# XinMing0411/AC-VAE

Hardware: AMD Instinct MI355X
Metric: train-step captions/s (and audio-sec/s) at B=32, 1/2/4/8 MI355X (higher is better)
Workload: dtype f32

## Files before the change

### acvae_amd/_lib.py

```python
import ctypes
import os
import re
import threading

import numpy as np
import torch

_HERE = os.path.dirname(os.path.abspath(__file__))
HEADER = os.path.join(os.path.dirname(_HERE), "include", "acvae_hip.h")
LIB_PATH = os.path.join(_HERE, "libacvae_hip.so")

_CT = {"int": ctypes.c_int, "int64_t": ctypes.c_int64, "float": ctypes.c_float, "double": ctypes.c_double,
       "uint64_t": ctypes.c_uint64}
ERRORS = {-1: "ACVAE_EINVAL (bad dims / null pointer)", -2: "ACVAE_EALIGN (alignment)",
          -3: "ACVAE_EUNSUPPORTED", -4: "ACVAE_EWORKSPACE (workspace too small)"}


def parse_header(path=HEADER):
    src = open(path).read()
    src = re.sub(r"/\*.*?\*/", "", src, flags=re.S)
    protos = {}
    for m in re.finditer(r"\b(int|int64_t)\s+(acvae_\w+)\s*\(([^)]*)\)\s*;", src):
        ret, name, args = m.group(1), m.group(2), m.group(3).strip()
        alist = []
# ... 3 lines not shown
                if "*" in a:
                    alist.append((a.split("*")[-1].strip(), ctypes.c_void_p))
                else:
                    toks = a.replace("const ", "").split()
                    alist.append((toks[-1], _CT[toks[0]]))
        protos[name] = (_CT[ret], alist)
    enums = {}
    for m in re.finditer(r"enum\s+\w*\s*\{([^}]*)\}", src):
        val = -1
        for item in m.group(1).split(","):
            item = item.strip()
            if not item:
                continue
            if "=" in item:
                k, v = item.split("=")
                val = int(v.strip(), 0)
                enums[k.strip()] = val
            else:
                val += 1
                enums[item] = val
    return protos, enums


PROTOS, ENUMS = parse_header()
_defs = dict(re.findall(r"#define\s+(ACVAE_\w+)\s+(\d+)", open(HEADER).read()))
ENUMS_TEXT_N = int(_defs["ACVAE_TEXT_NPARAMS"])
ENC_NPARAMS = int(_defs["ACVAE_ENC_NPARAMS"])
ENC_BF16 = int(_defs["ACVAE_ENC_BF16"])
FLAG_NO_PERSIST = int(_defs["ACVAE_FLAG_NO_PERSIST"])
FLAG_DEFER_PARAM_GRADS = int(_defs["ACVAE_FLAG_DEFER_PARAM_GRADS"])
FLAG_NO_ATTN_SPLIT = int(_defs["ACVAE_FLAG_NO_ATTN_SPLIT"])
FLAG_TEST_STALL = int(_defs["ACVAE_FLAG_TEST_STALL"])
FLAG_ROLLOUT_GRAD = int(_defs["ACVAE_FLAG_ROLLOUT_GRAD"])
_lib = None


class options:
    persist = os.environ.get("ACVAE_DECODE_PERSIST", "1") != "0"
    defer = os.environ.get("ACVAE_DECODE_DEFER", "1") != "0"
    attn_split = True
    test_stall = False


class override:
    _lock = threading.Lock()
    _open = []
    _base = None

    def __init__(self, **kw):
        self.kw = kw

    @staticmethod
    def _apply():
        vals = dict(override._base)
        for o in override._open:
            vals.update(o.kw)
        for k, v in vals.items():
            setattr(options, k, v)

    def __enter__(self):
        with override._lock:
            if not override._open:
                override._base = {k: v for k, v in vars(options).items() if not k.startswith("_")}
            override._open.append(self)
            override._apply()
        return self

    def __exit__(self, *exc):
        with override._lock:
            override._open.remove(self)
            override._apply()
        return False

# ... 180 lines not shown
```

### acvae_amd/csrc/decoder.hip

```cpp
#include <cstdlib>
#include <vector>
#include "common.h"
#include "conv.h"
#include "rnn.h"
#include "decode_persist.h"
#include "../../include/acvae_hip.h"

namespace {

struct Bump {
  long off = 0;
  long take(long n) { const long o = off; off = (off + n + 63) & ~63L; return o; }
};

struct Ctx {
  hipStream_t s;
  float* skws;
  operator hipStream_t() const { return s; }
};
inline int gemm(const float* A, long lda, const float* B, long ldb, const float* bias, float* C, long ldc, int M, int N,
                int K, int acc, const Ctx& st) {
  return acvae_gemm_nt_dual(A, lda, B, ldb, K, nullptr, 0, nullptr, 0, 0, bias, C, ldc, M, N, acc, st.s, st.skws);
}
inline int gemm2(const float* A1, long lda1, const float* B1, long ldb1, int K1, const float* A2, long lda2,
                 const float* B2, long ldb2, int K2, const float* bias, float* C, long ldc, int M, int N, int acc,
                 const Ctx& st) {
  if (M <= 64)
    return acvae_gemm_nt_dual(A1, lda1, B1, ldb1, K1, A2, lda2, B2, ldb2, K2, bias, C, ldc, M, N, acc, st.s, st.skws);
  ACVAE_TRY(acvae_gemm_nt_dual(A1, lda1, B1, ldb1, K1, nullptr, 0, nullptr, 0, 0, bias, C, ldc, M, N, acc, st.s, st.skws));
  return acvae_gemm_nt_dual(A2, lda2, B2, ldb2, K2, nullptr, 0, nullptr, 0, 0, nullptr, C, ldc, M, N, 1, st.s, st.skws);
}
struct TnWs { float* p; long bytes; };
inline int gemm_tn(const float* A, long lda, const float* B, long ldb, float* C, long ldc, int M, int N, int K, TnWs ws,
                   hipStream_t st) {
  return acvae_gemm_tn_fused(A, lda, B, ldb, C, ldc, M, N, K, 0, ws.p, ws.bytes, st);
}
inline void zb_skinny(acvae::ZeroBatch& zb, float* skws) { zb.add(skws, acvae_skinny_ticket_words()); }
inline void zb_colsum(acvae::ZeroBatch& zb, double* dpart) { zb.add(dpart, acvae::colsum_ticket_words()); }
inline void zb_tn(acvae::ZeroBatch& zb, TnWs ws) { zb.add(ws.p, TN_TICKETS); }
inline int transp(const float* in, long ld_in, float* out, long ld_out, int rows, int cols, hipStream_t st) {
  return acvae_transpose(in, ld_in, out, ld_out, rows, cols, st);
}
inline int zero(float* p, long n, hipStream_t st) {
  return hipMemsetAsync(p, 0, (size_t)n * sizeof(float), st) == hipSuccess ? ACVAE_OK : (int)hipGetLastError();
}
struct Fork {
  hipStream_t main_s, aux;
  bool on() const { return aux != main_s; }
  static int edge(hipStream_t from, hipStream_t to) {
    constexpr int RING = 64;
    struct Ring { hipEvent_t ev[RING]; int next; int dev; };
    static thread_local Ring ring = {{}, 0, -1};
    int dev = -1;
    if (hipGetDevice(&dev) != hipSuccess) return (int)hipGetLastError();
    if (dev != ring.dev) {
      for (int i = 0; i < RING; ++i) ring.ev[i] = nullptr;
      ring.next = 0; ring.dev = dev;
    }
    hipEvent_t& e = ring.ev[ring.next];
    ring.next = (ring.next + 1) % RING;
    if (!e && hipEventCreateWithFlags(&e, hipEventDisableTiming) != hipSuccess) return (int)hipGetLastError();
    hipError_t r = hipEventRecord(e, from);
    if (r == hipSuccess) r = hipStreamWaitEvent(to, e, 0);
    return r == hipSuccess ? ACVAE_OK : (int)r;
  }
  int begin() const { return on() ? edge(main_s, aux) : ACVAE_OK; }
  int join() const { return on() ? edge(aux, main_s) : ACVAE_OK; }
};
inline long tn_ws_floats(int M, int N, int K) { return acvae_gemm_tn_workspace_bytes(M, N, K) / 4 + 64 + TN_TICKETS; }

enum {
  TP_DEC_EMB, TP_DEC_WIH, TP_DEC_WHH, TP_DEC_BIH, TP_DEC_BHH, TP_DEC_CLS_W, TP_DEC_CLS_B, TP_DEC_ATT_V, TP_DEC_ATT_W,
  TP_DEC_ATT_B, TP_Q_EMB, TP_Q_WIH, TP_Q_WHH, TP_Q_BIH, TP_Q_BHH, TP_Q_WIH_R, TP_Q_WHH_R, TP_Q_BIH_R, TP_Q_BHH_R,
  TP_Q_TML_W, TP_Q_TML_B, TP_P_EMB, TP_P_ATT_V, TP_P_ATT_W, TP_P_ATT_B, TP_P_WIH, TP_P_WHH, TP_P_BIH, TP_P_BHH,
  TP_P_ML_W, TP_P_ML_B, TP_MLO_W, TP_MLO_B, TP_LN_W, TP_LN_B, TP_COUNT
};
static_assert(TP_COUNT == ACVAE_TEXT_NPARAMS, "text parameter table out of sync with the header");

constexpr int POST_MAX_LAYERS = 16;
struct PostLayout {
  long words, x, hidden[POST_MAX_LAYERS], save_f[POST_MAX_LAYERS], save_r[POST_MAX_LAYERS], hprev_f[POST_MAX_LAYERS],
      hprev_r[POST_MAX_LAYERS], argmax, saved_total;
  long gi_f, gi_r, gh, hf, ml, dml, dhid, dgi_f, dgi_r, dgh_f, dgh_r, dh_a, dh_b, dx, wt, wt2, wt_ih0, wt_ih1, wt_ml, pq_hbuf, pq_cnt, tn, dpart, skws,
       dhid2, wtu_hh0, wtu_hh1, wtu_ih0, wtu_ih1, scratch_total;
  long tn_floats, dpart_doubles, pq_cnt_words;
};
int post_layout(int N, int Tc, int E, int Hq, int V, int NL, PostLayout& L) {
  if (N <= 0 || Tc <= 0 || E <= 0 || Hq <= 0 || V <= 0 || NL < 1 || NL > POST_MAX_LAYERS) return ACVAE_EINVAL;
  const long R = (long)N * Tc;
  Bump s;
  L.words = s.take(R * 2);
  L.x = s.take(R * E);
  for (int k = 0; k < NL; ++k) {
    L.hidden[k] = s.take(R * 2 * Hq);
    L.save_f[k] = s.take(R * 4 * Hq); L.save_r[k] = s.take(R * 4 * Hq);
    L.hprev_f[k] = s.take(R * Hq); L.hprev_r[k] = s.take(R * Hq);
  }
  L.argmax = s.take((long)N * 2 * Hq);
  L.saved_total = s.off;
  Bump c;
  L.gi_f = c.take(R * 3 * Hq); L.gi_r = c.take(R * 3 * Hq);
// ... 1234 lines not shown
```

### acvae_amd/csrc/encoder.hip

```cpp
#include <algorithm>
#include "common.h"
#include "conv.h"
#include "resnet.h"
#include "../../include/acvae_hip.h"

namespace {

constexpr int kMaxBlocks = 6;
constexpr int kArchMask = 0xff;
constexpr int kChan[kMaxBlocks + 1] = {1, 64, 128, 256, 512, 1024, 2048};
struct Arch { int blocks; bool pool_last; };
inline bool arch_of(int arch, Arch& a) {
  if (arch & ~(kArchMask | ACVAE_ENC_BF16)) return false;
  if ((arch & kArchMask) == ACVAE_ARCH_CNN10) { a = {4, true}; return true; }
  if ((arch & kArchMask) == ACVAE_ARCH_CNN14_16K) { a = {6, false}; return true; }
  return false;
}
inline bool is_bf16(int arch) { return (arch & ACVAE_ENC_BF16) != 0; }
inline bool wino_on() {
  static const bool on = !getenv("ACVAE_CONV_WINO") || atoi(getenv("ACVAE_CONV_WINO")) != 0;
  return on;
}
template <class TA>
inline bool use_wino(int H, int W, int Cin, int Cout) {
  return sizeof(TA) == 4 && wino_on() && acvae::conv3x3_wino_ok(H, W, Cin, Cout);
}

struct EncLayout {
  int N, T, F;
  int nb, Cemb;
  bool pool[kMaxBlocks + 1];
  int H[kMaxBlocks + 1], W[kMaxBlocks + 1];
  long y1[kMaxBlocks + 1], y2[kMaxBlocks + 1], p[kMaxBlocks + 1];
  long wf1[kMaxBlocks + 1], wf2[kMaxBlocks + 1];
  long wd1[kMaxBlocks + 1], wd2[kMaxBlocks + 1];
  long bn[2 * kMaxBlocks + 1];
  long pooled_in;
  long total;
  long s_partials, s_dya, s_dyb, s_dpa, s_dpb, s_wd, s_slab, s_bnpart, s_c1w, s_c1b, s_dpart, s_total;
};

long align4(long x) { return (x + 63) & ~63L; }

int make_layout(int arch, int N, int T, int F, EncLayout& L) {
  Arch A;
  if (!arch_of(arch, A)) return ACVAE_EINVAL;
  const long esz = is_bf16(arch) ? 2 : 4;
  auto units = [esz](long n) { return (n * esz + 3) / 4; };
  const int div = 1 << (A.pool_last ? A.blocks : A.blocks - 1);
  if (N <= 0 || F != 64 || T < div) return ACVAE_EINVAL;
  L.N = N; L.T = T; L.F = F; L.nb = A.blocks; L.Cemb = kChan[A.blocks];
  long off = 0;
  int h = T, w = F;
  long max_act = 0, max_pool = 0, max_part = 0, max_slab = 0, max_bnpart = 0;
  for (int b = 1; b <= L.nb; ++b) {
    L.H[b] = h; L.W[b] = w;
    L.pool[b] = b < L.nb || A.pool_last;
    const long act = (long)N * h * w * kChan[b];
    const long pool = L.pool[b] ? (long)N * (h / 2) * (w / 2) * kChan[b] : act;
    L.y1[b] = off; off = align4(off + units(act));
    L.y2[b] = off; off = align4(off + units(act));
    L.p[b] = off; off = align4(off + units(pool));
    const long wtaps = esz == 4 ? 16 : 9;
    L.wf1[b] = off; off = align4(off + units((long)kChan[b] * wtaps * kChan[b - 1]));
    L.wf2[b] = off; off = align4(off + units((long)kChan[b] * wtaps * kChan[b]));
    L.wd1[b] = off; off = align4(off + units((long)kChan[b] * wtaps * kChan[b - 1]));
    L.wd2[b] = off; off = align4(off + units((long)kChan[b] * wtaps * kChan[b]));
    if (act > max_act) max_act = act;
    if (pool > max_pool) max_pool = pool;
    const long part = (long)acvae::conv_partials_rows(N, h, w) * 2 * kChan[b];
    if (part > max_part) max_part = part;
    if (w >= 4) {
// ... 15 lines not shown
      sl = esz == 2 ? acvae::conv3x3_wgrad_bf16_slab_floats(N, h, w, kChan[b - 1], kChan[b])
                    : acvae::conv3x3_wgrad_slab_floats(N, h, w, kChan[b - 1], kChan[b]);
      if (sl > max_slab) max_slab = sl;
    }
    long bp = (long)acvae::bn_bwd_blocks(N, h, w, kChan[b]) * 2 * kChan[b];
    if (esz == 4 && wino_on() && acvae::conv3x3_wino_ok(h, w, kChan[b], kChan[b]))
      bp = std::max(bp, (long)acvae::conv_wino_partials_rows(N, h, w) * 2 * kChan[b]);
    if (bp > max_bnpart) max_bnpart = bp;
    if (L.pool[b]) { h /= 2; w /= 2; }
  }
  L.H[0] = h; L.W[0] = w;
  for (int i = 0; i < 2 * L.nb + 1; ++i) {
    const int C = i == 0 ? 64 : kChan[(i - 1) / 2 + 1];
    L.bn[i] = off; off = align4(off + 4L * C);
  }
  L.pooled_in = off; off = align4(off + (long)N * L.Cemb);
  L.total = off;
  const long c1 = (long)acvae::conv1_first_blocks(N, T) * 128;
  const long b0 = (long)acvae::bn0_partials_rows((long)N * T) * 128;
  if (c1 > max_part) max_part = c1;
  if (b0 > max_part) max_part = b0;
  long s = 0;
  L.s_dpart = s; s = align4(s + 2 * acvae::colsum_scratch_doubles(2 * L.Cemb > 1024 ? 2 * L.Cemb : 1024));
  L.s_partials = s; s = align4(s + max_part);
  L.s_bnpart = s; s = align4(s + max_bnpart);
  L.s_wd = s; s = align4(s + units((long)L.Cemb * (esz == 4 ? 16 : 9) * L.Cemb));
  L.s_slab = s; s = align4(s + max_slab);
  L.s_c1w = s; s = align4(s + (long)acvae::conv1_first_blocks(N, T) * 576);
  L.s_c1b = s; s = align4(s + (long)acvae::conv1_first_blocks(N, T) * 128);
  L.s_dpa = s; s = align4(s + units(max_pool));
  L.s_dpb = s; s = align4(s + units(max_pool));
  L.s_dya = s; s = align4(s + units(max_act));
  L.s_dyb = s; s = align4(s + units(max_act));
  L.s_total = s;
  return ACVAE_OK;
}

inline int p_bn0(int k) { return k; }
inline int p_conv(int b, int which) { return 5 + (b - 1) * 12 + (which - 1); }
inline int p_bn(int b, int which, int k) { return 5 + (b - 1) * 12 + 2 + (which - 1) * 5 + k; }
inline int p_fc_w(int nb) { return 5 + nb * 12; }
inline int p_fc_b(int nb) { return 6 + nb * 12; }

template <class TA>
int conv_fwd(const TA* X, const float* scale, const float* shift, const float* W_oihw, float* wbuf, TA* Y, float* partials,
             int N, int H, int W, int Cin, int Cout, int* nparts, hipStream_t st, bool ready = false) {
  if constexpr (sizeof(TA) == 4) {
    if (use_wino<TA>(H, W, Cin, Cout)) {
      if (!ready) ACVAE_TRY(acvae::conv3x3_wino_weights(W_oihw, wbuf, Cout, Cin, false, st));
      *nparts = acvae::conv_wino_partials_rows(N, H, W);
      return acvae::conv3x3_wino(X, scale, shift, wbuf, Y, partials, N, H, W, Cin, Cout, st);
    }
  }
  if (!ready) ACVAE_TRY(acvae::repack_weights<TA>(W_oihw, (TA*)wbuf, nullptr, Cout, Cin, st));
  *nparts = acvae::conv_partials_rows(N, H, W);
  return acvae::conv3x3_igemm(X, scale, shift, (const TA*)wbuf, Y, partials, N, H, W, Cin, Cout, st);
}
template <class TA>
int conv_dgrad(const TA* dY, const float* W_oihw, TA* wbuf, TA* dX, int N, int H, int W, int Cin, int Cout, hipStream_t st,
               bool ready = false, const acvae::WinoBnReduce* red = nullptr, float* redpart = nullptr, int* red_rows = nullptr) {
  if (red_rows) *red_rows = 0;
  if constexpr (sizeof(TA) == 4) {
    if (use_wino<TA>(H, W, Cout, Cin)) {
      if (!ready) ACVAE_TRY(acvae::conv3x3_wino_weights(W_oihw, (float*)wbuf, Cout, Cin, true, st));
      const bool fuse = red && redpart && red_rows;
      if (fuse) *red_rows = acvae::conv_wino_partials_rows(N, H, W);
// ... 524 lines not shown
                                 const uint8_t* const* masks, void* stream) {
  if (is_r38(arch))
    return r38_fwd(params, feats, audio_embeds, pooled, saved_v, saved_bytes, scratch_v, scratch_bytes, arch, N, T, F, training,
                   p_block, p_fc, seed, masks, (hipStream_t)stream);
  if (is_bf16(arch))
    return encoder_fwd_t<bf16_t>(params, feats, audio_embeds, pooled, saved_v, saved_bytes, scratch_v, scratch_bytes, arch,
                                 N, T, F, training, p_block, p_fc, seed, masks, stream);
  return encoder_fwd_t<float>(params, feats, audio_embeds, pooled, saved_v, saved_bytes, scratch_v, scratch_bytes, arch, N,
                              T, F, training, p_block, p_fc, seed, masks, stream);
}

extern "C" int acvae_encoder_relu_mask(const void* saved_v, int64_t saved_bytes, int arch, int N, int T, int F, int site,
                                       uint8_t* mask_nchw, void* stream) {
  if (is_r38(arch)) return r38_relu_mask(saved_v, saved_bytes, arch, N, T, F, site, mask_nchw, (hipStream_t)stream);
  EncLayout L;
  ACVAE_TRY(make_layout(arch, N, T, F, L));
  if (!saved_v || !mask_nchw || site < 0 || site >= 2 * L.nb) return ACVAE_EINVAL;
  if (saved_bytes < L.total * (int64_t)sizeof(float)) return ACVAE_EWORKSPACE;
  float* saved = (float*)saved_v;
  const int b = site / 2 + 1, which = site % 2;
  BnPtrs bn = bn_at(saved, L, 1 + 2 * (b - 1) + which);
  const long off = which ? L.y2[b] : L.y1[b];
  if (is_bf16(arch))
    return acvae::relu_mask<bf16_t>((const bf16_t*)(saved + off), bn.scale, bn.shift, mask_nchw, N, L.H[b], L.W[b], kChan[b],
                                    (hipStream_t)stream);
  return acvae::relu_mask<float>(saved + off, bn.scale, bn.shift, mask_nchw, N, L.H[b], L.W[b], kChan[b], (hipStream_t)stream);
}

namespace {
template <class TA>
int encoder_bwd_t(const void* const* params, void* const* grads, const float* feats,
                                 const float* d_audio_embeds, void* saved_v, int64_t saved_bytes, void* scratch_v,
                                 int64_t scratch_bytes, int arch, int N, int T, int F, int training, float p_block,
                                 uint64_t seed, const uint8_t* const* masks, void* stream, void* block_done,
                                 void* user) {
  EncLayout L;
  ACVAE_TRY(make_layout(arch, N, T, F, L));
  if (!params || !grads || !feats || !d_audio_embeds || !saved_v || !scratch_v) return ACVAE_EINVAL;
  if (saved_bytes < L.total * (int64_t)sizeof(float) || scratch_bytes < L.s_total * (int64_t)sizeof(float))
    return ACVAE_EWORKSPACE;
  hipStream_t st = (hipStream_t)stream;
  float* saved = (float*)saved_v;
  float* scratch = (float*)scratch_v;
  auto P = [&](int i) { return (float*)params[i]; };
  auto G = [&](int i) { return (float*)grads[i]; };
  TA* dya = (TA*)(scratch + L.s_dya);
  TA* dyb = (TA*)(scratch + L.s_dyb);
  TA* dp_cur = (TA*)(scratch + L.s_dpa);
  TA* dp_nxt = (TA*)(scratch + L.s_dpb);
  TA* wd = (TA*)(scratch + L.s_wd);
  float* slab = scratch + L.s_slab;
  float* bnpart = scratch + L.s_bnpart;
  double* dpart = (double*)(scratch + L.s_dpart);
  const int S = L.H[0], Fp = L.W[0];
  ACVAE_TRY(acvae::colsum_tickets_reset(dpart, st));
  ACVAE_TRY(acvae::freq_mean_bwd<TA>(d_audio_embeds, dp_cur, (long)N * S, Fp, L.Cemb, st));
  for (int b = L.nb; b >= 1; --b) {
    const int H = L.H[b], W = L.W[b], C = kChan[b], Cin = kChan[b - 1];
    const TA* Y1 = (const TA*)(saved + L.y1[b]);
    const TA* Y2 = (const TA*)(saved + L.y2[b]);
    BnPtrs n1 = bn_at(saved, L, 1 + 2 * (b - 1)), n2 = bn_at(saved, L, 2 + 2 * (b - 1));
    ACVAE_TRY(acvae::bn_bwd<TA>(Y2, dp_cur, L.pool[b] ? UP_POOL : UP_DROP, n2.scale, n2.shift, n2.mean, n2.invstd, bnpart, G(p_bn(b, 2, 1)),
                            G(p_bn(b, 2, 0)), dya, dpart, N, H, W, C, dspec(p_block, masks, seed, b - 1, training), st,
                            training != 0));
    ACVAE_TRY(conv_wgrad<TA>((const TA*)dya, Y1, n1.scale, n1.shift, G(p_conv(b, 2)), slab, N, H, W, C, C, st));
    const bool wd_ready = training != 0;
    int red_rows = 0;
    acvae::WinoBnReduce red{(const float*)Y1, n1.scale, n1.shift, n1.mean, n1.invstd};
    ACVAE_TRY(conv_dgrad<TA>((const TA*)dya, P(p_conv(b, 2)), wd_ready ? (TA*)(saved + L.wd2[b]) : wd, dyb, N, H, W, C, C, st, wd_ready,
                             sizeof(TA) == 4 ? &red : nullptr, bnpart, &red_rows));
    DropoutSpec none{0.f, nullptr, 0, 0};
    const bool fold1 = b == 1 && sizeof(TA) == 4;
    if (fold1)
      ACVAE_TRY(acvae::bn_bwd_sums<TA>(Y1, dyb, UP_PLAIN, n1.scale, n1.shift, n1.mean, n1.invstd, bnpart, G(p_bn(b, 1, 1)),
                                       G(p_bn(b, 1, 0)), dpart, N, H, W, C, none, st, red_rows));
    else
      ACVAE_TRY(acvae::bn_bwd<TA>(Y1, dyb, UP_PLAIN, n1.scale, n1.shift, n1.mean, n1.invstd, bnpart, G(p_bn(b, 1, 1)),
                                  G(p_bn(b, 1, 0)), dya, dpart, N, H, W, C, none, st, training != 0, red_rows));
    if (b > 1) {
      ACVAE_TRY(conv_wgrad<TA>((const TA*)dya, (const TA*)(saved + L.p[b - 1]), nullptr, nullptr, G(p_conv(b, 1)), slab, N, H,
                               W, Cin, C, st));
      const bool fw = use_wino<TA>(H, W, Cin, C), dw = use_wino<TA>(H, W, C, Cin);
      const bool r1 = wd_ready && fw == dw;
      ACVAE_TRY(conv_dgrad<TA>((const TA*)dya, P(p_conv(b, 1)), r1 ? (TA*)(saved + L.wd1[b]) : wd, dp_nxt, N, H, W, Cin, C, st, r1));
      TA* t = dp_cur; dp_cur = dp_nxt; dp_nxt = t;
    } else {
      BnPtrs b0 = bn_at(saved, L, 0);
      const BnBwdApply a1{(const float*)Y1, n1.scale, n1.shift, n1.mean, n1.invstd, G(p_bn(1, 1, 1)), G(p_bn(1, 1, 0)),
                          bn_bwd_invn(N, H, W, training != 0)};
      ACVAE_TRY(acvae::conv1_first_bwd<TA>(feats, b0.scale, b0.shift, b0.mean, b0.invstd, P(p_conv(1, 1)),
                                           fold1 ? (const TA*)dyb : (const TA*)dya, scratch + L.s_c1w, scratch + L.s_c1b,
                                           G(p_conv(1, 1)), G(p_bn0(0)), G(p_bn0(1)), dpart, N, T, F, st,
                                           fold1 ? &a1 : nullptr));
    }
    if (block_done) ((void (*)(int, void*))block_done)(b, user);
  }
  return ACVAE_OK;
}
}

extern "C" int acvae_encoder_bwd_hooked(const void* const* params, void* const* grads, const float* feats,
                                 const float* d_audio_embeds, void* saved_v, int64_t saved_bytes, void* scratch_v,
                                 int64_t scratch_bytes, int arch, int N, int T, int F, int training, float p_block,
                                 uint64_t seed, const uint8_t* const* masks, void* stream, void* block_done,
                                 void* user) {
  if (is_r38(arch))
    return r38_bwd(params, grads, feats, d_audio_embeds, saved_v, saved_bytes, scratch_v, scratch_bytes, arch, N, T, F, training,
                   p_block, seed, masks, (hipStream_t)stream, block_done, user);
  if (is_bf16(arch))
    return encoder_bwd_t<bf16_t>(params, grads, feats, d_audio_embeds, saved_v, saved_bytes, scratch_v, scratch_bytes, arch,
                                 N, T, F, training, p_block, seed, masks, stream, block_done, user);
  return encoder_bwd_t<float>(params, grads, feats, d_audio_embeds, saved_v, saved_bytes, scratch_v, scratch_bytes, arch, N,
                              T, F, training, p_block, seed, masks, stream, block_done, user);
}

extern "C" int acvae_encoder_bwd(const void* const* params, void* const* grads, const float* feats,
                                 const float* d_audio_embeds, void* saved_v, int64_t saved_bytes, void* scratch_v,
                                 int64_t scratch_bytes, int arch, int N, int T, int F, int training, float p_block,
                                 uint64_t seed, const uint8_t* const* masks, void* stream) {
  return acvae_encoder_bwd_hooked(params, grads, feats, d_audio_embeds, saved_v, saved_bytes, scratch_v, scratch_bytes,
                                  arch, N, T, F, training, p_block, seed, masks, stream, nullptr, nullptr);
}
```

### acvae_amd/encoder.py

```python
import ctypes

import torch
import torch.nn as nn

from . import _lib

_SCRATCH = {}
_BLOCK_HOOK = ctypes.CFUNCTYPE(None, ctypes.c_int, ctypes.c_void_p)


def scratch_buffer(nbytes, device, tag=None):
    key = (device.type, device.index, torch.cuda.current_stream(device).cuda_stream, tag)
    buf = _SCRATCH.get(key)
    if buf is None or buf.numel() < nbytes:
        _SCRATCH[key] = buf = torch.empty(int(nbytes), dtype=torch.uint8, device=device)
    return buf


def ptr_table(tensors):
    return (ctypes.c_void_p * len(tensors))(*[None if t is None else t.data_ptr() for t in tensors])


def init_layer(layer):
    nn.init.xavier_uniform_(layer.weight)
# ... 52 lines not shown
        seed = mod._next_seed() if training else 0
        mt = ptr_table(masks) if masks is not None else None
        _lib.call("acvae_encoder_fwd", ptr_table(tensors), feats, ae, pooled, saved, saved_b, scratch, scratch_b, arch,
                  N, T, F, int(training), float(mod.p_block), float(mod.p_fc), seed, mt, _lib.current_stream())
        ctx.mod, ctx.feats, ctx.saved, ctx.masks, ctx.seed, ctx.training = mod, feats, saved, masks, seed, training
        ctx.arch = arch
        if mod.keep_saved:
            mod._last_saved = (saved, arch, N, T, F)
        ctx.mark_non_differentiable(pooled)
        return ae, pooled

    @staticmethod
    def backward(ctx, d_ae, _d_pooled):
        mod, feats = ctx.mod, ctx.feats
        N, T, F = feats.shape
        tensors = mod._param_table()
        grads = [None] * len(tensors)
        outs = []
        for i, t in enumerate(tensors):
            if t.dtype.is_floating_point and t.requires_grad and i < len(tensors) - 2:
                grads[i] = mod._grad_buffer(t)
        d_ae = d_ae.contiguous().float()
        scratch_b = _lib.call("acvae_encoder_scratch_bytes", ctx.arch, N, T, F)
        scratch = scratch_buffer(scratch_b, feats.device)
        mt = ptr_table(ctx.masks) if ctx.masks is not None else None
        hook, failed = None, []
        if mod._grad_ready_cb is not None:
            def block_done(block, _user):
                try:
                    mod._grad_ready_cb(("encoder_block", int(block)))
                except BaseException as exc:
                    failed.append(exc)
            hook = _BLOCK_HOOK(block_done)
        _lib.call("acvae_encoder_bwd_hooked", ptr_table(tensors), ptr_table(grads), feats, d_ae, ctx.saved,
                  ctx.saved.numel(), scratch, scratch_b, ctx.arch, N, T, F, int(ctx.training), float(mod.p_block), ctx.seed, mt,
                  _lib.current_stream(), ctypes.cast(hook, ctypes.c_void_p) if hook is not None else None, None)
        if failed:
            raise failed[0]
        ctx.saved = None
        if mod._grad_ready_cb is not None:
            mod._grad_ready_cb("encoder")
        for w in mod._weights():
            outs.append(next((g for t, g in zip(tensors, grads) if t is w), None))
        return (None, None, *outs)


class _PannsCnn(nn.Module):
    ARCH, N_BLOCKS, TIME_DIV, OUT_CHANNELS, HEAD = 0, 4, 16, 512, "embed_pooled"

    def __init__(self, inputdim, embed_size, **kwargs):
        super().__init__()
        self.inputdim = inputdim
        self.embed_size = embed_size
        self.bn0 = nn.BatchNorm2d(64)
        chans = [1, 64, 128, 256, 512, 1024, 2048]
        for b in range(1, self.N_BLOCKS + 1):
            setattr(self, f"conv_block{b}", ConvBlock(chans[b - 1], chans[b]))
        setattr(self, self.HEAD, nn.Linear(self.OUT_CHANNELS, self.OUT_CHANNELS, bias=True))
        init_bn(self.bn0)
        init_layer(getattr(self, self.HEAD))
        self.p_block, self.p_fc = 0.2, 0.5
        self.compute_dtype = kwargs.get("compute_dtype", "f32")
        self.dropout_masks = None
        self._seed_base, self._calls = None, 0
        self.keep_saved = False
        self._last_saved = None
        self._grad_views = None
        self._grad_ready_cb = None

    def _arch(self):
        if self.compute_dtype not in ("f32", "bf16"):
            raise ValueError(f"compute_dtype must be 'f32' or 'bf16', not {self.compute_dtype!r}")
        return self.ARCH | (_lib.ENC_BF16 if self.compute_dtype == "bf16" else 0)

    def _blocks(self):
        return [getattr(self, f"conv_block{b}") for b in range(1, self.N_BLOCKS + 1)]

    def _n_dropout_sites(self):
        return self.N_BLOCKS + 2

    def _deep_block(self):
        return getattr(self, f"conv_block{self.N_BLOCKS}"), self.N_BLOCKS

    def _head(self):
        return getattr(self, self.HEAD)

    def _param_table(self):
        t = _bn_tensors(self.bn0)
        for blk in self._blocks():
            t += [blk.conv1.weight, blk.conv2.weight] + _bn_tensors(blk.bn1) + _bn_tensors(blk.bn2)
        t += [self._head().weight, self._head().bias]
        return t

    def _weights(self):
        return [t for t in self._param_table()[:-2] if isinstance(t, nn.Parameter)]

    def _grad_buffer(self, p):
        if self._grad_views is not None and p in self._grad_views:
            return self._grad_views[p].detach()
        return torch.empty_like(p)

# ... 66 lines not shown
                                           nn.BatchNorm2d(planes))
                init_layer(downsample[1]); init_bn(downsample[2])
            blocks = [_ResnetBasicBlock(inplanes, planes, stride, downsample)]
            inplanes = planes
            blocks += [_ResnetBasicBlock(inplanes, planes) for _ in range(1, n)]
            setattr(self, f"layer{i + 1}", nn.Sequential(*blocks))

    def blocks(self):
        return [b for i in range(1, 5) for b in getattr(self, f"layer{i}")]


class ResNet38(_PannsCnn):
    ARCH, N_BLOCKS, TIME_DIV, OUT_CHANNELS, HEAD = 2, 0, 32, 2048, "fc1"

    def __init__(self, inputdim, embed_size, **kwargs):
        nn.Module.__init__(self)
        self.inputdim = inputdim
        self.embed_size = embed_size
        self.bn0 = nn.BatchNorm2d(64)
        self.conv_block1 = ConvBlock(1, 64)
        self.resnet = _ResNet()
        self.conv_block_after1 = ConvBlock(512, 2048)
        self.fc1 = nn.Linear(2048, 2048)
        init_bn(self.bn0)
        init_layer(self.fc1)
        self.p_block, self.p_fc = 0.2, 0.5
        self.compute_dtype = kwargs.get("compute_dtype", "f32")
        self.dropout_masks = None
        self._seed_base, self._calls = None, 0
        self.keep_saved = False
        self._last_saved = None
        self._grad_views = None
        self._grad_ready_cb = None

    def _arch(self):
        if self.compute_dtype != "f32":
            raise ValueError(f"ResNet38 runs in fp32 only (compute_dtype={self.compute_dtype!r})")
        return self.ARCH

    def _n_dropout_sites(self):
        return 21

    def _deep_block(self):
        return self.conv_block_after1, 0

    def _param_table(self):
        t = _bn_tensors(self.bn0)
        cb = self.conv_block1
        t += [cb.conv1.weight, cb.conv2.weight] + _bn_tensors(cb.bn1) + _bn_tensors(cb.bn2)
        for blk in self.resnet.blocks():
            t += [blk.conv1.weight] + _bn_tensors(blk.bn1) + [blk.conv2.weight] + _bn_tensors(blk.bn2)
            if blk.downsample is not None:
                t += [blk.downsample[1].weight] + _bn_tensors(blk.downsample[2])
        ca = self.conv_block_after1
        t += [ca.conv1.weight, ca.conv2.weight] + _bn_tensors(ca.bn1) + _bn_tensors(ca.bn2)
        t += [self.fc1.weight, self.fc1.bias]
        return t

    def site_shapes(self, N, T):
        relu, drop = [], []
        h, w = T, 64
        relu += [(N, 64, h, w)] * 2
        h, w = h // 2, w // 2
        drop.append((N, 64, h, w))
        for blk in self.resnet.blocks():
            if blk.stride == 2:
# ... 20 lines not shown
```

### acvae_amd/vae_model.py

```python
import contextlib
import os
import random
import weakref

import numpy as np
import torch
import torch.nn as nn

from . import _lib, text_encoder
from .encoder import ptr_table, scratch_buffer
from .word_model import CaptionModel


class _DecodeFn(torch.autograd.Function):
    @staticmethod
    def forward(ctx, model, mem, mem_lens_d, caps_d, lens1_d, q_z, eps_p, ss_flags, dis_flags, Tc, sampling, *weights):
        N, S, Eenc = mem.shape
        dec = model.decoder
        E, H, A, V = dec.embed_size, dec.model.hidden_size, dec.attn.attn_size, dec.vocab_size
        dev = mem.device
        train = caps_d is not None
        params = model._text_table()
        dims = (N, Tc, S, E, H, A, V, Eenc)
        saved_b = _lib.call("acvae_decode_saved_bytes", *dims)
# ... 74 lines not shown
            else:
                ev_aux = torch.cuda.Event()
                ev_aux.record(model._side_stream(torch.cuda.current_stream()))
                model._grad_ready_cb("decode_deferred", (ev, ev_aux))
        if defers:
            side, cur = model._side_stream(torch.cuda.current_stream()), torch.cuda.current_stream()
            for t in [ctx.saved, outputs, d_qz, mem] + [u for u in ups if u is not None]:
                t.record_stream(side)
            if any(p is not None and p.is_leaf and p.grad is not None for p in params):
                cur.wait_stream(side)
            else:
                torch.autograd.Variable._execution_engine.queue_callback(lambda: cur.wait_stream(side))
        ctx.saved = None
        outs = [next((g for p, g in zip(params, grads) if p is w), None) for w in model._decode_weights()]
        return (None, d_mem, None, None, None, d_qz, None, None, None, None, None, *outs)


class Hybrid_VAEModel(CaptionModel):
    def __init__(self, Audioencoder: nn.Module, Textdecoder: nn.Module, **kwargs):
        super().__init__(Audioencoder, Textdecoder, **kwargs)
        E = Textdecoder.embed_size
        self.qnet = getattr(text_encoder, kwargs["posterior_model"])(
            word_dim=E, embed_size=E, vocab_size=Textdecoder.vocab_size, **kwargs["posterior_args"])
        self.pnet = getattr(text_encoder, kwargs["prior_model"])(
            word_dim=E, audiofeats_size=E, embed_size=E, vocab_size=Textdecoder.vocab_size, **kwargs["prior_args"])
        self.mean_log_out = nn.Linear(E, 2 * E)
        if E != Audioencoder.embed_size:
            self.ln = nn.Linear(Audioencoder.embed_size, E)
            nn.init.xavier_uniform_(self.ln.weight)
        nn.init.xavier_uniform_(self.mean_log_out.weight)
        self.qnet._owner = weakref.ref(self)
        self.pnet._owner = weakref.ref(self)
        self.decoder._owner = weakref.ref(self)
        self._encproj_cache = {}
        self.use_side_stream = os.environ.get("ACVAE_SIDE_STREAM", "1") != "0"
        self.defer_param_grads = True
        self.staged = None
        self.noise = None
        self._grad_views = None
        self._grad_ready_cb = None

    def _text_table(self):
        d, q, p = self.decoder, self.qnet, self.pnet
        g, qn, pn = d.model, q.network, p.network
        t = [d.embedding_table(), g.weight_ih_l0, g.weight_hh_l0, g.bias_ih_l0, g.bias_hh_l0,
             d.classifier.weight, d.classifier.bias, d.attn.v, d.attn.h2attn.weight, d.attn.h2attn.bias,
             q.word_embedding.weight, qn.weight_ih_l0, qn.weight_hh_l0, qn.bias_ih_l0, qn.bias_hh_l0,
             qn.weight_ih_l0_reverse, qn.weight_hh_l0_reverse, qn.bias_ih_l0_reverse, qn.bias_hh_l0_reverse,
             q.token_mean_log.weight, q.token_mean_log.bias,
             p.word_embedding.weight, p.word_attn.v, p.word_attn.h2attn.weight, p.word_attn.h2attn.bias,
             pn.weight_ih_l0, pn.weight_hh_l0, pn.bias_ih_l0, pn.bias_hh_l0, p.mean_log_out.weight, p.mean_log_out.bias,
             self.mean_log_out.weight, self.mean_log_out.bias]
        t += [self.ln.weight, self.ln.bias] if hasattr(self, "ln") else [None, None]
        assert len(t) == _lib.ENUMS_TEXT_N
        return t

    def _decode_weights(self):
        t = self._text_table()
        return [p for i, p in enumerate(t) if p is not None and (i < 10 or i >= 21)]

    def _grad_buffer(self, p):
        if self._grad_views is not None and p in self._grad_views:
            return self._grad_views[p].detach()
        return torch.empty_like(p)

    def _set_grad_views(self, views):
# ... 321 lines not shown
```

### include/acvae_hip.h

```cpp
#ifndef ACVAE_HIP_H
#define ACVAE_HIP_H
#include <stdint.h>
#ifdef __cplusplus
extern "C" {
#endif

#define ACVAE_ABI_VERSION 3
int acvae_abi_version(void);

#define ACVAE_FLAG_NO_PERSIST 1
#define ACVAE_FLAG_DEFER_PARAM_GRADS 2
#define ACVAE_FLAG_NO_ATTN_SPLIT 4
#define ACVAE_FLAG_ROLLOUT_GRAD 16
#define ACVAE_FLAG_TEST_STALL 8

int acvae_persist_status_register(int device, void* status_words_host);

int acvae_gemm_nt(const float* A, int64_t lda, const float* B, int64_t ldb, const float* bias, float* C,
                  int64_t ldc, int M, int N, int K, int accumulate, void* stream);
int acvae_gemm_tn(const float* A, int64_t lda, const float* B, int64_t ldb, float* C, int64_t ldc, int M, int N,
                  int K, int accumulate, float* slab_ws, int64_t slab_ws_bytes, void* stream);
int64_t acvae_gemm_tn_workspace_bytes(int M, int N, int K);
int64_t acvae_colsum_workspace_bytes(int cols);
int acvae_colsum(const float* x, int rows, int cols, float* out, void* ws, int64_t ws_bytes, void* stream);

int64_t acvae_gemm_nt_splitk_workspace_bytes(void);
int acvae_gemm_nt_split_plan(int M, int N, int K1, int K2, int with_ws);
int acvae_gemm_nt_dual_ws(const float* A1, int64_t lda1, const float* B1, int64_t ldb1, int K1, const float* A2,
                          int64_t lda2, const float* B2, int64_t ldb2, int K2, const float* bias, float* C, int64_t ldc,
                          int M, int N, int accumulate, float* ws, int64_t ws_bytes, int reset_tickets, void* stream);
int acvae_gemm_nt_pair_c(const float* A0, int64_t lda0, const float* B0, int64_t ldb0, int K0, const float* bias0, float* C0,
                         int64_t ldc0, int N0, int acc0, const float* A1, int64_t lda1, const float* B1, int64_t ldb1, int K1,
                         const float* bias1, float* C1, int64_t ldc1, int N1, int acc1, int M, void* stream);
int64_t acvae_gemm_tn_fused_workspace_bytes(int M, int N, int K);
int acvae_gemm_tn_fused_plan(int M, int N, int K, int64_t ws_bytes);
int acvae_gemm_tn_fused_c(const float* A, int64_t lda, const float* B, int64_t ldb, float* C, int64_t ldc, int M, int N,
                          int K, int accumulate, float* ws, int64_t ws_bytes, int reset_tickets, void* stream);
int64_t acvae_colsum_batch_workspace_bytes(int n, const int* P, const int* width);
int acvae_colsum_batch_plan(int n, const int* P, const int* width, int64_t ws_bytes);
int acvae_colsum_batch(int n, const void* const* x, const int* P, const int* width, const void* const* out,
                       const void* const* out_b, void* ws, int64_t ws_bytes, int reset_tickets, void* stream);
int acvae_transpose(const float* in, int64_t ld_in, float* out, int64_t ld_out, int rows, int cols, void* stream);

int64_t acvae_attn_fwd_workspace_bytes(int N, int Tq, int S, int A, int E);
int acvae_attn_fwd(const float* qproj, int64_t q_sn, int64_t q_sj, const float* encproj, const float* enc,
                   const int64_t* lens, const float* v, float* ctx, int64_t c_sn, int64_t c_sj, float* weights,
// ... 44 lines not shown
                        double log_d, const uint64_t* ref_keys, const double* ref_w, int n_entries, const int* ref_off,
                        const double* ref_norm, const int* ref_len, int n_refs, const int* doc_ref, int n_docs,
                        const int* row_doc, const int* row_src, const double* len_factor, int n_len, double* score,
                        void* stream);
int acvae_ciderd_reward(const double* score, int n, int sample_n, float* reward, double* reward_mean, void* stream);
int acvae_mse_fwd(const float* a, const float* b, float* partials, float* out_scalar, int64_t n, void* stream);
int acvae_mse_bwd(const float* a, const float* b, const float* grad_out, float* da, float* db, int64_t n, void* stream);
int acvae_loss_combine_fwd(const float* ce, const float* kl, const float* mse, float w_kl, float w_mse, float* out, void* stream);
int acvae_loss_combine_bwd(const float* grad_out, float w_kl, float w_mse, float* g_ce, float* g_kl, float* g_mse, void* stream);

#define ACVAE_ENC_NPARAMS 55
#define ACVAE_ARCH_CNN10 0
#define ACVAE_ARCH_CNN14_16K 1
#define ACVAE_ARCH_RESNET38 2
#define ACVAE_ENC_BF16 256
int acvae_encoder_nparams(int arch);
int acvae_encoder_out_dims(int arch, int T, int* S, int* C);
int64_t acvae_encoder_saved_bytes(int arch, int N, int T, int F);
int64_t acvae_encoder_scratch_bytes(int arch, int N, int T, int F);
int acvae_encoder_fwd(const void* const* params, const float* feats, float* audio_embeds, float* pooled,
                      void* saved, int64_t saved_bytes, void* scratch, int64_t scratch_bytes, int arch, int N, int T,
                      int F, int training, float p_block, float p_fc, uint64_t seed, const uint8_t* const* masks,
                      void* stream);
int acvae_encoder_bwd(const void* const* params, void* const* grads, const float* feats,
                      const float* d_audio_embeds, void* saved, int64_t saved_bytes, void* scratch,
                      int64_t scratch_bytes, int arch, int N, int T, int F, int training, float p_block, uint64_t seed,
                      const uint8_t* const* masks, void* stream);
int acvae_encoder_relu_mask(const void* saved, int64_t saved_bytes, int arch, int N, int T, int F, int site,
                            uint8_t* mask_nchw, void* stream);
int acvae_encoder_bwd_hooked(const void* const* params, void* const* grads, const float* feats,
                             const float* d_audio_embeds, void* saved, int64_t saved_bytes, void* scratch,
                             int64_t scratch_bytes, int arch, int N, int T, int F, int training, float p_block,
                             uint64_t seed, const uint8_t* const* masks, void* stream, void* block_done, void* user);

int64_t acvae_conv3x3_workspace_bytes(int N, int H, int W, int Cin, int Cout);
int acvae_conv3x3_fwd(const float* X, const float* W_oihw, const float* in_scale, const float* in_shift, float* Y,
                      const float* gamma, const float* beta, float* running_mean, float* running_var,
                      int64_t* num_batches_tracked, int training, float* bn_out, void* ws, int64_t ws_bytes, int N, int H,
                      int W, int Cin, int Cout, void* stream);
int acvae_conv3x3_dgrad(const float* dY, const float* W_oihw, float* dX, void* ws, int64_t ws_bytes, int N, int H, int W,
                        int Cin, int Cout, void* stream);
int acvae_conv3x3_wgrad(const float* dY, const float* X, const float* in_scale, const float* in_shift, float* dW_oihw,
                        void* ws, int64_t ws_bytes, int N, int H, int W, int Cin, int Cout, void* stream);
int acvae_conv1_first_bwd(const float* x, const float* bn0, const float* W1_oihw, const float* dY, float* dW1,
                          float* dgamma0, float* dbeta0, void* ws, int64_t ws_bytes, int N, int T, int F, void* stream);
int acvae_conv1_first_bwd_bn(const float* x, const float* bn0, const float* W1_oihw, const float* Y1, const float* dO,
                             const float* bn1, float* dgamma1, float* dbeta1, float* dW1, float* dgamma0, float* dbeta0,
                             void* ws, int64_t ws_bytes, int N, int T, int F, int training, void* stream);
int acvae_conv3x3_fwd_wino(const float* X, const float* W_oihw, const float* in_scale, const float* in_shift, float* Y,
                           const float* gamma, const float* beta, float* running_mean, float* running_var,
                           int64_t* num_batches_tracked, int training, float* bn_out, void* ws, int64_t ws_bytes, int N,
                           int H, int W, int Cin, int Cout, void* stream);
int acvae_conv3x3_dgrad_wino(const float* dY, const float* W_oihw, float* dX, void* ws, int64_t ws_bytes, int N, int H,
                             int W, int Cin, int Cout, void* stream);
int acvae_conv3x3_dgrad_bnred_wino(const float* dY, const float* W_oihw, float* dX, const float* Yprev, const float* bn_prev,
                                   float* sum_g, float* sum_gy, void* ws, int64_t ws_bytes, int N, int H, int W, int Cin,
                                   int Cout, void* stream);
int acvae_conv3x3_wgrad_wino(const float* dY, const float* X, const float* in_scale, const float* in_shift, float* dW_oihw,
                             void* ws, int64_t ws_bytes, int N, int H, int W, int Cin, int Cout, void* stream);
int acvae_conv3x3_fwd_bf16(const void* X, const float* W_oihw, const float* in_scale, const float* in_shift, void* Y,
                           const float* gamma, const float* beta, float* running_mean, float* running_var,
                           int64_t* num_batches_tracked, int training, float* bn_out, void* ws, int64_t ws_bytes, int N,
                           int H, int W, int Cin, int Cout, void* stream);
int acvae_conv3x3_dgrad_bf16(const void* dY, const float* W_oihw, void* dX, void* ws, int64_t ws_bytes, int N, int H, int W,
                             int Cin, int Cout, void* stream);
int acvae_conv3x3_wgrad_bf16(const void* dY, const void* X, const float* in_scale, const float* in_shift, float* dW_oihw,
// ... 158 lines not shown
```

Before: 2116.

## Overlap encoder conv weight-gradient kernels on an aux stream during backward

Moves the conv wgrad kernels of the encoder backward onto the model's auxiliary stream so they run concurrently with the dgrad/bn_bwd critical path on the main stream. The single dZ buffer becomes a three-slot ring, and events gate when a slot can be reused. Block-done callbacks are reordered so a block is announced only after its weight gradients finish. This adds scratch memory and event overhead, and with the shared slab workspace concurrent wgrads could contend for resources.

```diff
diff --git a/acvae_amd/_lib.py b/acvae_amd/_lib.py
--- a/acvae_amd/_lib.py
+++ b/acvae_amd/_lib.py
@@ -59,6 +59,7 @@
 FLAG_NO_ATTN_SPLIT = int(_defs["ACVAE_FLAG_NO_ATTN_SPLIT"])
 FLAG_TEST_STALL = int(_defs["ACVAE_FLAG_TEST_STALL"])
 FLAG_ROLLOUT_GRAD = int(_defs["ACVAE_FLAG_ROLLOUT_GRAD"])
+FLAG_ENC_BWD_INORDER = int(_defs["ACVAE_FLAG_ENC_BWD_INORDER"])
 _lib = None
 
 
@@ -66,6 +67,7 @@
     persist = os.environ.get("ACVAE_DECODE_PERSIST", "1") != "0"
     defer = os.environ.get("ACVAE_DECODE_DEFER", "1") != "0"
     attn_split = True
+    enc_bwd = os.environ.get("ACVAE_ENC_BWD", "streams")
     test_stall = False
 
 
diff --git a/acvae_amd/csrc/decoder.hip b/acvae_amd/csrc/decoder.hip
--- a/acvae_amd/csrc/decoder.hip
+++ b/acvae_amd/csrc/decoder.hip
@@ -4,6 +4,7 @@
 #include "conv.h"
 #include "rnn.h"
 #include "decode_persist.h"
+#include "stream_fork.h"
 #include "../../include/acvae_hip.h"
 
 namespace {
@@ -44,29 +45,7 @@
 inline int zero(float* p, long n, hipStream_t st) {
   return hipMemsetAsync(p, 0, (size_t)n * sizeof(float), st) == hipSuccess ? ACVAE_OK : (int)hipGetLastError();
 }
-struct Fork {
-  hipStream_t main_s, aux;
-  bool on() const { return aux != main_s; }
-  static int edge(hipStream_t from, hipStream_t to) {
-    constexpr int RING = 64;
-    struct Ring { hipEvent_t ev[RING]; int next; int dev; };
-    static thread_local Ring ring = {{}, 0, -1};
-    int dev = -1;
-    if (hipGetDevice(&dev) != hipSuccess) return (int)hipGetLastError();
-    if (dev != ring.dev) {
-      for (int i = 0; i < RING; ++i) ring.ev[i] = nullptr;
-      ring.next = 0; ring.dev = dev;
-    }
-    hipEvent_t& e = ring.ev[ring.next];
-    ring.next = (ring.next + 1) % RING;
-    if (!e && hipEventCreateWithFlags(&e, hipEventDisableTiming) != hipSuccess) return (int)hipGetLastError();
-    hipError_t r = hipEventRecord(e, from);
-    if (r == hipSuccess) r = hipStreamWaitEvent(to, e, 0);
-    return r == hipSuccess ? ACVAE_OK : (int)r;
-  }
-  int begin() const { return on() ? edge(main_s, aux) : ACVAE_OK; }
-  int join() const { return on() ? edge(aux, main_s) : ACVAE_OK; }
-};
+using acvae::Fork;
 inline long tn_ws_floats(int M, int N, int K) { return acvae_gemm_tn_workspace_bytes(M, N, K) / 4 + 64 + TN_TICKETS; }
 
 enum {
diff --git a/acvae_amd/csrc/encoder.hip b/acvae_amd/csrc/encoder.hip
--- a/acvae_amd/csrc/encoder.hip
+++ b/acvae_amd/csrc/encoder.hip
@@ -2,6 +2,7 @@
 #include "common.h"
 #include "conv.h"
 #include "resnet.h"
+#include "stream_fork.h"
 #include "../../include/acvae_hip.h"
 
 namespace {
@@ -37,7 +38,7 @@
   long bn[2 * kMaxBlocks + 1];
   long pooled_in;
   long total;
-  long s_partials, s_dya, s_dyb, s_dpa, s_dpb, s_wd, s_slab, s_bnpart, s_c1w, s_c1b, s_dpart, s_total;
+  long s_partials, s_dya, s_dyb, s_dyc, s_dyd, s_dpa, s_dpb, s_wd, s_slab, s_bnpart, s_c1w, s_c1b, s_dpart, s_total;
 };
 
 long align4(long x) { return (x + 63) & ~63L; }
@@ -119,6 +120,8 @@
   L.s_dpb = s; s = align4(s + units(max_pool));
   L.s_dya = s; s = align4(s + units(max_act));
   L.s_dyb = s; s = align4(s + units(max_act));
+  L.s_dyc = s; s = align4(s + units(max_act));
+  L.s_dyd = s; s = align4(s + units(max_act));
   L.s_total = s;
   return ACVAE_OK;
 }
@@ -709,19 +712,22 @@
 int encoder_bwd_t(const void* const* params, void* const* grads, const float* feats,
                                  const float* d_audio_embeds, void* saved_v, int64_t saved_bytes, void* scratch_v,
                                  int64_t scratch_bytes, int arch, int N, int T, int F, int training, float p_block,
-                                 uint64_t seed, const uint8_t* const* masks, void* stream, void* block_done,
-                                 void* user) {
+                                 uint64_t seed, const uint8_t* const* masks, void* stream, void* aux_stream, void* block_done,
+                                 void* user, int flags) {
+  using acvae::Fork;
   EncLayout L;
   ACVAE_TRY(make_layout(arch, N, T, F, L));
   if (!params || !grads || !feats || !d_audio_embeds || !saved_v || !scratch_v) return ACVAE_EINVAL;
   if (saved_bytes < L.total * (int64_t)sizeof(float) || scratch_bytes < L.s_total * (int64_t)sizeof(float))
     return ACVAE_EWORKSPACE;
   hipStream_t st = (hipStream_t)stream;
+  const bool inorder = (flags & ACVAE_FLAG_ENC_BWD_INORDER) != 0;
+  hipStream_t ws = (!inorder && aux_stream && aux_stream != stream) ? (hipStream_t)aux_stream : st;
+  const bool two = ws != st;
   float* saved = (float*)saved_v;
   float* scratch = (float*)scratch_v;
   auto P = [&](int i) { return (float*)params[i]; };
   auto G = [&](int i) { return (float*)grads[i]; };
-  TA* dya = (TA*)(scratch + L.s_dya);
   TA* dyb = (TA*)(scratch + L.s_dyb);
   TA* dp_cur = (TA*)(scratch + L.s_dpa);
   TA* dp_nxt = (TA*)(scratch + L.s_dpb);
@@ -729,6 +735,30 @@
   float* slab = scratch + L.s_slab;
   float* bnpart = scratch + L.s_bnpart;
   double* dpart = (double*)(scratch + L.s_dpart);
+  TA* dz[3] = {(TA*)(scratch + L.s_dya), (TA*)(scratch + L.s_dyc), (TA*)(scratch + L.s_dyd)};
+  hipEvent_t zfree[3] = {nullptr, nullptr, nullptr};
+  const int nz = inorder ? 1 : 3;
+  int taken = 0;
+  auto take = [&](int* slot) -> int {
+    *slot = taken++ % nz;
+    if (zfree[*slot]) ACVAE_TRY(Fork::after(st, zfree[*slot]));
+    zfree[*slot] = nullptr;
+    return ACVAE_OK;
+  };
+  struct WJob { const TA* dY; const TA* X; const float* scale; const float* shift; float* dW; int H, W, Cin, Cout, slot; hipEvent_t ready; };
+  hipEvent_t last_w = nullptr;
+  auto ready = [&](WJob& j) -> int { return two ? Fork::mark(st, &j.ready) : ACVAE_OK; };
+  auto wgrad = [&](const WJob& j) -> int {
+    if (two) ACVAE_TRY(Fork::after(ws, j.ready));
+    ACVAE_TRY(conv_wgrad<TA>(j.dY, j.X, j.scale, j.shift, j.dW, slab, N, j.H, j.W, j.Cin, j.Cout, ws));
+    if (two) { ACVAE_TRY(Fork::mark(ws, &last_w)); zfree[j.slot] = last_w; }
+    return ACVAE_OK;
+  };
+  auto announce = [&](int b) -> int {
+    if (two && last_w && (block_done || b == 1)) ACVAE_TRY(Fork::after(st, last_w));
+    if (block_done) ((void (*)(int, void*))block_done)(b, user);
+    return ACVAE_OK;
+  };
   const int S = L.H[0], Fp = L.W[0];
   ACVAE_TRY(acvae::colsum_tickets_reset(dpart, st));
   ACVAE_TRY(acvae::freq_mean_bwd<TA>(d_audio_embeds, dp_cur, (long)N * S, Fp, L.Cemb, st));
@@ -737,43 +767,77 @@
     const TA* Y1 = (const TA*)(saved + L.y1[b]);
     const TA* Y2 = (const TA*)(saved + L.y2[b]);
     BnPtrs n1 = bn_at(saved, L, 1 + 2 * (b - 1)), n2 = bn_at(saved, L, 2 + 2 * (b - 1));
+    int s2 = 0;
+    ACVAE_TRY(take(&s2));
+    TA* dZ2 = dz[s2];
     ACVAE_TRY(acvae::bn_bwd<TA>(Y2, dp_cur, L.pool[b] ? UP_POOL : UP_DROP, n2.scale, n2.shift, n2.mean, n2.invstd, bnpart, G(p_bn(b, 2, 1)),
-                            G(p_bn(b, 2, 0)), dya, dpart, N, H, W, C, dspec(p_block, masks, seed, b - 1, training), st,
+                            G(p_bn(b, 2, 0)), dZ2, dpart, N, H, W, C, dspec(p_block, masks, seed, b - 1, training), st,
                             training != 0));
-    ACVAE_TRY(conv_wgrad<TA>((const TA*)dya, Y1, n1.scale, n1.shift, G(p_conv(b, 2)), slab, N, H, W, C, C, st));
+    WJob w2{dZ2, Y1, n1.scale, n1.shift, G(p_conv(b, 2)), H, W, C, C, s2, nullptr};
+    ACVAE_TRY(ready(w2));
+    if (inorder) ACVAE_TRY(wgrad(w2));
     const bool wd_ready = training != 0;
     int red_rows = 0;
     acvae::WinoBnReduce red{(const float*)Y1, n1.scale, n1.shift, n1.mean, n1.invstd};
-    ACVAE_TRY(conv_dgrad<TA>((const TA*)dya, P(p_conv(b, 2)), wd_ready ? (TA*)(saved + L.wd2[b]) : wd, dyb, N, H, W, C, C, st, wd_ready,
+    ACVAE_TRY(conv_dgrad<TA>((const TA*)dZ2, P(p_conv(b, 2)), wd_ready ? (TA*)(saved + L.wd2[b]) : wd, dyb, N, H, W, C, C, st, wd_ready,
                              sizeof(TA) == 4 ? &red : nullptr, bnpart, &red_rows));
     DropoutSpec none{0.f, nullptr, 0, 0};
     const bool fold1 = b == 1 && sizeof(TA) == 4;
-    if (fold1)
+    TA* dZ1 = nullptr;
+    int s1 = 0;
+    if (fold1) {
       ACVAE_TRY(acvae::bn_bwd_sums<TA>(Y1, dyb, UP_PLAIN, n1.scale, n1.shift, n1.mean, n1.invstd, bnpart, G(p_bn(b, 1, 1)),
                                        G(p_bn(b, 1, 0)), dpart, N, H, W, C, none, st, red_rows));
-    else
+    } else {
+      ACVAE_TRY(take(&s1));
+      dZ1 = dz[s1];
       ACVAE_TRY(acvae::bn_bwd<TA>(Y1, dyb, UP_PLAIN, n1.scale, n1.shift, n1.mean, n1.invstd, bnpart, G(p_bn(b, 1, 1)),
-                                  G(p_bn(b, 1, 0)), dya, dpart, N, H, W, C, none, st, training != 0, red_rows));
+                                  G(p_bn(b, 1, 0)), dZ1, dpart, N, H, W, C, none, st, training != 0, red_rows));
+    }
+    WJob w1{dZ1, (const TA*)(saved + L.p[b - 1]), nullptr, nullptr, G(p_conv(b, 1)), H, W, Cin, C, s1, nullptr};
     if (b > 1) {
-      ACVAE_TRY(conv_wgrad<TA>((const TA*)dya, (const TA*)(saved + L.p[b - 1]), nullptr, nullptr, G(p_conv(b, 1)), slab, N, H,
-                               W, Cin, C, st));
+      ACVAE_TRY(ready(w1));
+      if (inorder) ACVAE_TRY(wgrad(w1));
       const bool fw = use_wino<TA>(H, W, Cin, C), dw = use_wino<TA>(H, W, C, Cin);
       const bool r1 = wd_ready && fw == dw;
-      ACVAE_TRY(conv_dgrad<TA>((const TA*)dya, P(p_conv(b, 1)), r1 ? (TA*)(saved + L.wd1[b]) : wd, dp_nxt, N, H, W, Cin, C, st, r1));
+      ACVAE_TRY(conv_dgrad<TA>((const TA*)dZ1, P(p_conv(b, 1)), r1 ? (TA*)(saved + L.wd1[b]) : wd, dp_nxt, N, H, W, Cin, C, st, r1));
       TA* t = dp_cur; dp_cur = dp_nxt; dp_nxt = t;
     } else {
       BnPtrs b0 = bn_at(saved, L, 0);
       const BnBwdApply a1{(const float*)Y1, n1.scale, n1.shift, n1.mean, n1.invstd, G(p_bn(1, 1, 1)), G(p_bn(1, 1, 0)),
                           bn_bwd_invn(N, H, W, training != 0)};
       ACVAE_TRY(acvae::conv1_first_bwd<TA>(feats, b0.scale, b0.shift, b0.mean, b0.invstd, P(p_conv(1, 1)),
-                                           fold1 ? (const TA*)dyb : (const TA*)dya, scratch + L.s_c1w, scratch + L.s_c1b,
+                                           fold1 ? (const TA*)dyb : (const TA*)dZ1, scratch + L.s_c1w, scratch + L.s_c1b,
                                            G(p_conv(1, 1)), G(p_bn0(0)), G(p_bn0(1)), dpart, N, T, F, st,
                                            fold1 ? &a1 : nullptr));
     }
-    if (block_done) ((void (*)(int, void*))block_done)(b, user);
-  }
+    if (inorder) {
+      ACVAE_TRY(announce(b));
+      continue;
+    }
+    if (b < L.nb) ACVAE_TRY(announce(b + 1));
+    ACVAE_TRY(wgrad(w2));
+    if (b > 1) ACVAE_TRY(wgrad(w1));
+  }
+  if (!inorder) ACVAE_TRY(announce(1));
   return ACVAE_OK;
 }
+}
+
+extern "C" int acvae_encoder_bwd_streams(const void* const* params, void* const* grads, const float* feats,
+                                 const float* d_audio_embeds, void* saved_v, int64_t saved_bytes, void* scratch_v,
+                                 int64_t scratch_bytes, int arch, int N, int T, int F, int training, float p_block,
+                                 uint64_t seed, const uint8_t* const* masks, void* stream, void* aux_stream,
+                                 void* block_done, void* user, int flags) {
+  if (flags & ~ACVAE_FLAG_ENC_BWD_INORDER) return ACVAE_EINVAL;
+  if (is_r38(arch))
+    return r38_bwd(params, grads, feats, d_audio_embeds, saved_v, saved_bytes, scratch_v, scratch_bytes, arch, N, T, F, training,
+                   p_block, seed, masks, (hipStream_t)stream, block_done, user);
+  if (is_bf16(arch))
+    return encoder_bwd_t<bf16_t>(params, grads, feats, d_audio_embeds, saved_v, saved_bytes, scratch_v, scratch_bytes, arch,
+                                 N, T, F, training, p_block, seed, masks, stream, aux_stream, block_done, user, flags);
+  return encoder_bwd_t<float>(params, grads, feats, d_audio_embeds, saved_v, saved_bytes, scratch_v, scratch_bytes, arch, N,
+                              T, F, training, p_block, seed, masks, stream, aux_stream, block_done, user, flags);
 }
 
 extern "C" int acvae_encoder_bwd_hooked(const void* const* params, void* const* grads, const float* feats,
@@ -781,14 +845,8 @@
                                  int64_t scratch_bytes, int arch, int N, int T, int F, int training, float p_block,
                                  uint64_t seed, const uint8_t* const* masks, void* stream, void* block_done,
                                  void* user) {
-  if (is_r38(arch))
-    return r38_bwd(params, grads, feats, d_audio_embeds, saved_v, saved_bytes, scratch_v, scratch_bytes, arch, N, T, F, training,
-                   p_block, seed, masks, (hipStream_t)stream, block_done, user);
-  if (is_bf16(arch))
-    return encoder_bwd_t<bf16_t>(params, grads, feats, d_audio_embeds, saved_v, saved_bytes, scratch_v, scratch_bytes, arch,
-                                 N, T, F, training, p_block, seed, masks, stream, block_done, user);
-  return encoder_bwd_t<float>(params, grads, feats, d_audio_embeds, saved_v, saved_bytes, scratch_v, scratch_bytes, arch, N,
-                              T, F, training, p_block, seed, masks, stream, block_done, user);
+  return acvae_encoder_bwd_streams(params, grads, feats, d_audio_embeds, saved_v, saved_bytes, scratch_v, scratch_bytes, arch,
+                                   N, T, F, training, p_block, seed, masks, stream, nullptr, block_done, user, 0);
 }
 
 extern "C" int acvae_encoder_bwd(const void* const* params, void* const* grads, const float* feats,
diff --git a/acvae_amd/csrc/stream_fork.h b/acvae_amd/csrc/stream_fork.h
--- /dev/null
+++ b/acvae_amd/csrc/stream_fork.h
@@ -0,0 +1,38 @@
+#pragma once
+#include <hip/hip_runtime.h>
+#include "../../include/acvae_hip.h"
+
+namespace acvae {
+struct Fork {
+  hipStream_t main_s, aux;
+  bool on() const { return aux != main_s; }
+  static constexpr int RING = 64;
+  static int mark(hipStream_t from, hipEvent_t* out) {
+    struct Ring { hipEvent_t ev[RING]; int next; int dev; };
+    static thread_local Ring ring = {{}, 0, -1};
+    int dev = -1;
+    if (hipGetDevice(&dev) != hipSuccess) return (int)hipGetLastError();
+    if (dev != ring.dev) {
+      for (int i = 0; i < RING; ++i) ring.ev[i] = nullptr;
+      ring.next = 0; ring.dev = dev;
+    }
+    hipEvent_t& e = ring.ev[ring.next];
+    ring.next = (ring.next + 1) % RING;
+    if (!e && hipEventCreateWithFlags(&e, hipEventDisableTiming) != hipSuccess) return (int)hipGetLastError();
+    const hipError_t r = hipEventRecord(e, from);
+    *out = e;
+    return r == hipSuccess ? ACVAE_OK : (int)r;
+  }
+  static int after(hipStream_t to, hipEvent_t e) {
+    const hipError_t r = hipStreamWaitEvent(to, e, 0);
+    return r == hipSuccess ? ACVAE_OK : (int)r;
+  }
+  static int edge(hipStream_t from, hipStream_t to) {
+    hipEvent_t e = nullptr;
+    const int r = mark(from, &e);
+    return r != ACVAE_OK ? r : after(to, e);
+  }
+  int begin() const { return on() ? edge(main_s, aux) : ACVAE_OK; }
+  int join() const { return on() ? edge(aux, main_s) : ACVAE_OK; }
+};
+}
diff --git a/acvae_amd/encoder.py b/acvae_amd/encoder.py
--- a/acvae_amd/encoder.py
+++ b/acvae_amd/encoder.py
@@ -108,9 +108,13 @@
                 except BaseException as exc:
                     failed.append(exc)
             hook = _BLOCK_HOOK(block_done)
-        _lib.call("acvae_encoder_bwd_hooked", ptr_table(tensors), ptr_table(grads), feats, d_ae, ctx.saved,
+        mode = _lib.options.enc_bwd
+        owner = mod._owner() if mod._owner is not None else None
+        aux = owner._aux_stream() if mode == "streams" and owner is not None else None
+        _lib.call("acvae_encoder_bwd_streams", ptr_table(tensors), ptr_table(grads), feats, d_ae, ctx.saved,
                   ctx.saved.numel(), scratch, scratch_b, ctx.arch, N, T, F, int(ctx.training), float(mod.p_block), ctx.seed, mt,
-                  _lib.current_stream(), ctypes.cast(hook, ctypes.c_void_p) if hook is not None else None, None)
+                  _lib.current_stream(), aux, ctypes.cast(hook, ctypes.c_void_p) if hook is not None else None, None,
+                  _lib.FLAG_ENC_BWD_INORDER if mode == "inorder" else 0)
         if failed:
             raise failed[0]
         ctx.saved = None
@@ -143,6 +147,7 @@
         self._last_saved = None
         self._grad_views = None
         self._grad_ready_cb = None
+        self._owner = None
 
     def _arch(self):
         if self.compute_dtype not in ("f32", "bf16"):
@@ -275,6 +280,7 @@
         self._last_saved = None
         self._grad_views = None
         self._grad_ready_cb = None
+        self._owner = None
 
     def _arch(self):
         if self.compute_dtype != "f32":
diff --git a/acvae_amd/vae_model.py b/acvae_amd/vae_model.py
--- a/acvae_amd/vae_model.py
+++ b/acvae_amd/vae_model.py
@@ -130,6 +130,8 @@
         self.qnet._owner = weakref.ref(self)
         self.pnet._owner = weakref.ref(self)
         self.decoder._owner = weakref.ref(self)
+        if hasattr(self.encoder, "_owner"):
+            self.encoder._owner = weakref.ref(self)
         self._encproj_cache = {}
         self.use_side_stream = os.environ.get("ACVAE_SIDE_STREAM", "1") != "0"
         self.defer_param_grads = True
diff --git a/include/acvae_hip.h b/include/acvae_hip.h
--- a/include/acvae_hip.h
+++ b/include/acvae_hip.h
@@ -12,6 +12,7 @@
 #define ACVAE_FLAG_DEFER_PARAM_GRADS 2
 #define ACVAE_FLAG_NO_ATTN_SPLIT 4
 #define ACVAE_FLAG_ROLLOUT_GRAD 16
+#define ACVAE_FLAG_ENC_BWD_INORDER 32
 #define ACVAE_FLAG_TEST_STALL 8
 
 int acvae_persist_status_register(int device, void* status_words_host);
@@ -122,6 +123,11 @@
                              const float* d_audio_embeds, void* saved, int64_t saved_bytes, void* scratch,
                              int64_t scratch_bytes, int arch, int N, int T, int F, int training, float p_block,
                              uint64_t seed, const uint8_t* const* masks, void* stream, void* block_done, void* user);
+int acvae_encoder_bwd_streams(const void* const* params, void* const* grads, const float* feats,
+                              const float* d_audio_embeds, void* saved, int64_t saved_bytes, void* scratch,
+                              int64_t scratch_bytes, int arch, int N, int T, int F, int training, float p_block,
+                              uint64_t seed, const uint8_t* const* masks, void* stream, void* aux_stream, void* block_done,
+                              void* user, int flags);
 
 int64_t acvae_conv3x3_workspace_bytes(int N, int H, int W, int Cin, int Cout);
 int acvae_conv3x3_fwd(const float* X, const float* W_oihw, const float* in_scale, const float* in_shift, float* Y,
```

After: 2133 (median of 6 runs). About the same (+0.8%).
